# r9y9/wavenet_vocoder

Hardware: NVIDIA H100
Metric: audio samples/sec (22.05 kHz MoL, 24-layer) (higher is better)
Workload: dtype f32

## Files before the change

wavenet_vocoder_b200/csrc/wn_host.cu:

```cuda
#include <cuda_runtime.h>
#include <stdint.h>
#include <stdio.h>
#include <stdlib.h>
#include <string.h>
#include <math.h>

#include <algorithm>
#include <string>
#include <vector>

#include "../../include/wn.h"
#include "wn_plan.h"
#include "wn_kernel.cuh"
#include "wn7_plan.h"
#include "wn7_kernel.cuh"
#include "wn_aux.cuh"
#include "wn_dense.cuh"

static thread_local std::string g_err;
static int32_t fail(int32_t code, const std::string& msg) {
    g_err = msg;
    return code;
}
#define CUDA_TRY(expr)                                                                          \
// ... 108 lines not shown
    o = 0;
    pl.tb_Td = o;  o += pl.NQ_D * pl.R * 4;
    pl.tb_Sk = o;  o += pl.NQ_BS * pl.G2 * 4;
    pl.tb_sb = o;  o += 4 * pl.NQ_BS;
    pl.tb_Ha = o;  o += pl.NQ_HA * pl.S * 4;
    pl.tb_Hab = o; o += 4 * pl.NQ_HA;
    pl.tb_Hb = o;  o += pl.NQ_HB * pl.S * 4;
    pl.tb_Hbb = o; o += 4 * pl.NQ_HB;
    pl.tb_floats = align_up(o, 4);
    pl.slot_floats = align_up(std::max(pl.fb_floats, std::max(pl.L > 1 ? pl.lb_floats : 0, pl.tb_floats)), 32);
    pl.cta_w_floats = (long long)pl.fb_floats + (long long)(pl.L - 1) * pl.lb_floats + pl.tb_floats;
    pl.nblobs = pl.L + 1;
    pl.cta_cw_floats = (long long)pl.L * pl.NQ_A * pl.C * 4;

    pl.NE = pl.L + 3;
    int nc = c.exchange_copies > 0 ? c.exchange_copies : env_int("WN_NCOPY", 0);
    const int max_items = std::max(std::max(pl.NYm, pl.NXm), std::max(pl.NSm, std::max(pl.NAm, pl.NBm))) * BT;
    if (max_items > 64) return fail(WN_ERR_INVALID, "too many rows per block for this batch tile (use more blocks)");
    if (nc <= 0) nc = 1;
    nc = std::min(nc, 64 / max_items);
    pl.ncopy = std::max(1, std::min(nc, P));
    if ((pl.G2 & 1) || (pl.R & 1) || (pl.S & 1))
        return fail(WN_ERR_INVALID, "residual, gate/2 and skip channel counts must be even (16-byte exchange loads)");
    pl.ex_yx = 0;
    pl.ex_sk = pl.L * (pl.G2 + pl.R);
    pl.ex_h1 = pl.ex_sk + pl.S;
    pl.ex_h2 = pl.ex_h1 + pl.S;
    pl.ex_elems = pl.ex_h2 + pl.O;
    pl.xc_shift = env_int("WN_XC_SHIFT", 5);
    pl.xstride = env_int("WN_XSTRIDE", WN_XSTRIDE);
    pl.copy_stride_pairs = ((((long long)pl.ex_elems * BT) >> pl.xc_shift) + 2) * pl.xstride + 96;

    ringtab.assign((size_t)pl.L * std::max(pl.kw - 1, 0) * 2, 0);
    long long pos = 0;
    for (int l = 0; l < pl.L; ++l)
        for (int k = 0; k < pl.kw - 1; ++k) {
            const int D = (pl.kw - 1 - k) * wn_dilation(pl, l);
            ringtab[((size_t)l * (pl.kw - 1) + k) * 2] = (int)pos;
            ringtab[((size_t)l * (pl.kw - 1) + k) * 2 + 1] = D;
            pos += D;
        }
    pl.ring_pos_total = pos;
    const long long ring_bytes = pos * pl.RA4 * BT * 4;

    auto layout = [&](bool ring_smem) -> long long {
        long long off = 0;
        auto take = [&](long long bytes, int al) {
            off = ((off + al - 1) / al) * al;
            long long r = off;
            off += bytes;
            return (int)r;
        };
        pl.sm_bar = take((long long)(2 * pl.nblobs + 8) * 8, 16);
        pl.sm_misc = take(16, 16);
        pl.sm_in = take((long long)BT * 8 + (pl.input_kind == WN_INPUT_ONEHOT ? (long long)BT * pl.O * 4 : 0), 16);
        pl.sm_ringtab = take((long long)ringtab.size() / 2 * 3 * 4 + 16, 16);
        pl.sm_xs = take(2LL * (pl.R + pl.G2) * BT * 4, 16);
        const int nq1 = std::max(pl.NQ_A + pl.NQ_BO, std::max(pl.NQ_BS, std::max(pl.NQ_HA, pl.NQ_HB)));
        pl.red1_floats = nq1 * 4 * BT * 4 + 4;
        pl.sm_red1 = take(2LL * pl.red1_floats * 4, 16);
        pl.red2_floats = (pl.NQ_D + pl.NQ_BS + pl.NQ_BO) * 4 * BT * 4 + 4;
        pl.sm_red2 = take(2LL * pl.red2_floats * 4, 16);
        pl.sm_sb = take(2LL * pl.L * pl.RA4 * BT * 4, 16);
        pl.sm_cond = take(pl.C > 0 ? 2LL * pl.L * pl.RA4 * BT * 4 : 16, 16);
        pl.sm_skipacc = take((long long)(pl.NSm * BT + 8 * pl.NQ_BS) * 4 + 16, 16);
        pl.sm_hs = take((long long)pl.O * BT * 4, 16);
        pl.sm_noise = take((long long)BT * (pl.O + 2) * 4, 16);
        pl.sm_first = take(2LL * pl.R * 4, 16);
        pl.sm_ring = take(ring_smem ? ring_bytes : 16, 16);
        pl.sm_slots = take(0, 128);
        return off;
    };
    const long long slot_bytes = (long long)pl.slot_floats * 4;
    const int want_ring_smem = env_int("WN_RING_SMEM", -1);
    bool ring_smem = (want_ring_smem != 0) && ring_bytes <= 96 * 1024;
    long long fixed = layout(ring_smem);
    long long fit = (smem_cap - fixed) / slot_bytes;
    if (ring_smem && want_ring_smem < 0 && fit < std::min<long long>(pl.nblobs, 3)) {
        ring_smem = false;
        fixed = layout(false);
        fit = (smem_cap - fixed) / slot_bytes;
    }
    pl.ring_in_smem = ring_smem ? 1 : 0;
    if (fit >= pl.nblobs) {
        pl.nres = pl.nblobs;
        pl.nring = 0;
    } else {
        if (fit < 2) return fail(WN_ERR_INVALID, "shared memory too small for two weight slots (use more blocks)");
        int nr = c.ring_slots > 0 ? c.ring_slots : env_int("WN_RING_SLOTS", 4);
        nr = (int)std::max<long long>(2, std::min<long long>(nr, fit));
        pl.nring = nr;
        pl.nres = (int)fit - nr;
        const int force_res = env_int("WN_RESIDENT", -1);
        if (force_res >= 0 && force_res < pl.nres) pl.nres = force_res;
    }
    pl.smem_bytes = (int)(pl.sm_slots + (long long)(pl.nres + pl.nring) * slot_bytes);
    if (pl.smem_bytes > smem_cap) return fail(WN_ERR_INVALID, "shared memory map exceeds the per-block limit");
    return WN_OK;
}

static void fill_work(const wn_config& c, wn_plan_info* out) {
    const int64_t R = c.residual_channels, G = c.gate_channels, G2 = G / 2, S = c.skip_channels, O = c.out_channels;
    const int64_t L = c.layers, kw = c.kernel_size, C = c.cin_channels;
    const int64_t cin0 = (c.input_kind == WN_INPUT_SCALAR) ? 1 : O;
    const int64_t mac = cin0 * R + L * (G * kw * R + G * C + S * G2 + R * G2) + S * S + O * S;
    const int64_t biases = R + L * (G + S + R) + S + O;
    out->flops_per_sample = 2 * mac;
    out->weight_bytes_per_step = 4 * (mac + biases);
}

static void fill_info(const wn_config& c, const WnPlan& pl, wn_plan_info* out) {
    memset(out, 0, sizeof(*out));
    out->num_ctas = pl.P;
    out->threads_per_cta = WN_NTHREADS;
    out->batch_tile = pl.BT;
    out->rows_y = pl.NYm;
    out->rows_x = pl.NXm;
    out->rows_skip = pl.NSm;
    out->rows_head_a = pl.NAm;
    out->rows_head_b = pl.NBm;
// ... 1580 lines not shown
```

wavenet_vocoder_b200/csrc/wn_kernel.cuh:

```cuda
#pragma once
#include <cuda_runtime.h>
#include <stdint.h>
#include <math.h>
#include "wn_plan.h"

struct WnPtrs {
    const float* wpack;
    const float* cwpack;
    const float* gbias;
    const float* first_w;
    const float* first_b;
    uint2* xbuf;
    float* ring_g;
    const int* ringtab;
    int* err;
    const float* c;
    const float* initial;
    const float* initial_dense;
    const int* initial_rows;
    const float* test_scalar;
    const int* test_index;
    const float* test_dense;
    const float* u1;
    const float* u2;
// ... 167 lines not shown
            for (int i = 0; i < NV / 2; ++i) {
                if (i < n) {
                    const float send = hi ? v[i] : v[i + n];
                    const float keep = hi ? v[i + n] : v[i];
                    v[i] = keep + __shfl_xor_sync(0xffffffffu, send, off);
                }
            }
        } else {
            v[0] += __shfl_xor_sync(0xffffffffu, v[0], off);
        }
    }
}

__host__ __device__ constexpr int ilog2c(int v) { return v <= 1 ? 0 : 1 + ilog2c(v >> 1); }

__device__ __forceinline__ uint4 philox4(uint4 ctr, uint2 key) {
#pragma unroll
    for (int r = 0; r < 10; ++r) {
        const uint32_t hi0 = __umulhi(0xD2511F53u, ctr.x), lo0 = 0xD2511F53u * ctr.x;
        const uint32_t hi1 = __umulhi(0xCD9E8D57u, ctr.z), lo1 = 0xCD9E8D57u * ctr.z;
        ctr = make_uint4(hi1 ^ ctr.y ^ key.x, lo1, hi0 ^ ctr.w ^ key.y, lo0);
        key.x += 0x9E3779B9u;
        key.y += 0xBB67AE85u;
    }
    return ctr;
}
__device__ __forceinline__ float u01(uint32_t r) {
    const float u = ((r >> 8) + 0.5f) * (1.0f / 16777216.0f);
    return 1e-5f + u * (1.0f - 2e-5f);
}


__device__ __noinline__ long long wn_check_abort(volatile int* s_abort, int* err, long long timeout, uint32_t what,
                                                 int p, long long t0) {
    if (*s_abort) return -1;
    if (ld_flag(err) != 0) {
        *s_abort = 1;
        return -1;
    }
    const long long now = clock64();
    if (t0 == 0) return now;
    if (now - t0 > timeout) {
        if (atomicCAS(err, 0, 1) == 0) {
            err[1] = (int)what;
            err[2] = p;
            err[3] = (int)threadIdx.x;
        }
        *s_abort = 1;
        return -1;
    }
    return t0;
}

#define WN_PROF_SLOTS 96
enum { WN_PC_ACQ, WN_PC_POLL, WN_PC_STASH, WN_PC_FMA, WN_PC_READY, WN_PC_REDUCE, WN_PC_STORE, WN_PC_BAR, WN_PC_FIN,
       WN_PC_PUB, WN_PC_DDONE, WN_PC_HEAD, WN_PC_TAIL, WN_PC_CRIT };
enum { WN_PD_WAIT, WN_PD_UNSTASH, WN_PD_GEMV, WN_PD_BAR, WN_PD_FIN, WN_PD_REST, WN_PC_DEF };
enum { WN_PS_SKEW = 4 * WN_PC_CRIT, WN_PS_DEF = WN_PS_SKEW + 6, WN_PS_TMA = WN_PS_DEF + 4 * WN_PC_DEF,
       WN_PS_COND = WN_PS_TMA + 2 };
static_assert(WN_PS_COND + 2 <= WN_PROF_SLOTS, "stage profile slots");
#ifdef WN_STAGE_PROF
#define WN_PROF_DECL(N) const bool prof_ = (pp.prof != nullptr) && lane == 0; long long pc_[N] = {}, tc_ = 0;
#define WN_PROF_START() if (prof_) tc_ = clock64();
#define WN_TICK(i) if (prof_) { const long long now_ = clock64(); pc_[i] += now_ - tc_; tc_ = now_; }
#define WN_TICK_AFTER(i, sink, v) if (prof_) { *reinterpret_cast<volatile float*>(sink) = (v); } WN_TICK(i)
#define WN_PROF_STORE(base, N) if (prof_) { for (int i_ = 0; i_ < (N); ++i_) pp.prof[(size_t)p * WN_PROF_SLOTS + (base) + i_] = pc_[i_]; }
#else
#define WN_PROF_DECL(N)
#define WN_PROF_START()
#define WN_TICK(i)
#define WN_TICK_AFTER(i, sink, v)
#define WN_PROF_STORE(base, N)
#endif

#define WN_NTC 128
#define WN_GW 4
#define WN_DISPATCH_E(EV, ...)                                \
    switch (EV) {                                             \
        case 1: { constexpr int E = 1; __VA_ARGS__ } break;   \
        case 2: { constexpr int E = 2; __VA_ARGS__ } break;   \
        case 4: { constexpr int E = 4; __VA_ARGS__ } break;   \
        default: { constexpr int E = 8; __VA_ARGS__ } break;  \
    }

template <int BT, int ER, int EG, bool STREAM = false>
struct Engine {
    static constexpr int NV = 4 * BT;
    static constexpr int NA = (BT >= 8) ? 1 : 2;
    const WnPlan& pl;
    const WnPtrs& pp;
    unsigned char* sm;
    int tid, warp, lane, p;
    int gt, gw;
    uint64_t *bar_full, *bar_empty, *bar_cfull, *bar_cempty;
    volatile int* s_abort;
    volatile int* s_stash_cnt;
    volatile int* s_ddone_cnt;
    int* ringtab;
    float *xs, *ys, *red1, *red2, *sb, *pre, *cond, *skipacc, *hs, *noise, *first, *slots;
    volatile float* ring;
    float* s_in;
    int* s_idx;
    float* s_dense;
    bool dead;

    __device__ Engine(const WnPlan& pl_, const WnPtrs& pp_, unsigned char* sm_)
        : pl(pl_), pp(pp_), sm(sm_) {
        lane = threadIdx.x & 31;
        warp = pp.warp_reverse ? (WN_NTHREADS / 32 - 1) - (int)(threadIdx.x >> 5) : (int)(threadIdx.x >> 5);
        tid = warp * 32 + lane;
        p = blockIdx.x;
        gt = tid & (WN_NTC - 1);
        gw = warp & (WN_GW - 1);
        const int nslots = pl.nres + pl.nring;
        bar_full = reinterpret_cast<uint64_t*>(sm + pl.sm_bar);
        bar_empty = bar_full + nslots;
        bar_cfull = bar_empty + (pl.nring > 0 ? pl.nring : 1);
        bar_cempty = bar_cfull + 2;
        s_abort = reinterpret_cast<volatile int*>(sm + pl.sm_misc);
        s_stash_cnt = s_abort + 1;
        s_ddone_cnt = s_abort + 2;
        s_in = reinterpret_cast<float*>(sm + pl.sm_in);
        s_idx = reinterpret_cast<int*>(s_in + BT);
        s_dense = reinterpret_cast<float*>(s_idx + BT);
        ringtab = reinterpret_cast<int*>(sm + pl.sm_ringtab);
        xs = reinterpret_cast<float*>(sm + pl.sm_xs);
        ys = xs + 2 * pl.R * BT;
        red1 = reinterpret_cast<float*>(sm + pl.sm_red1);
        red2 = reinterpret_cast<float*>(sm + pl.sm_red2);
        sb = reinterpret_cast<float*>(sm + pl.sm_sb);
        pre = sb + (size_t)pl.L * pl.RA4 * BT;
        cond = reinterpret_cast<float*>(sm + pl.sm_cond);
        skipacc = reinterpret_cast<float*>(sm + pl.sm_skipacc);
        hs = reinterpret_cast<float*>(sm + pl.sm_hs);
        noise = reinterpret_cast<float*>(sm + pl.sm_noise);
        first = reinterpret_cast<float*>(sm + pl.sm_first);
        slots = reinterpret_cast<float*>(sm + pl.sm_slots);
        if (pl.ring_in_smem)
            ring = reinterpret_cast<volatile float*>(sm + pl.sm_ring);
        else
            ring = pp.ring_g + (size_t)p * pl.ring_pos_total * pl.RA4 * BT;
        dead = false;
    }

    __device__ __forceinline__ bool check_abort(uint32_t what, long long& t0) {
        t0 = wn_check_abort(s_abort, pp.err, pp.timeout_cycles, what, p, t0);
        return t0 < 0;
    }
    template <bool relaxed = false>
    __device__ __forceinline__ bool wait_bar(uint64_t* bar, uint32_t parity, uint32_t what) {
        uint32_t spins = 0;
        long long t0 = 0;
        while (!mbar_try_wait(bar, parity)) {
            if (relaxed) __nanosleep(64);
            if (((++spins) & (relaxed ? 63u : 255u)) == 0 && check_abort(what, t0)) return false;
        }
        return true;
    }
    template <bool relaxed = false>
    __device__ __forceinline__ void wait_count(volatile int* cnt, int need, uint32_t what) {
        uint32_t spins = 0;
        long long t0 = 0;
        while (*cnt < need) {
            if (relaxed) __nanosleep(32);
            if (((++spins) & (relaxed ? 63u : 255u)) == 0 && check_abort(what, t0)) {
                dead = true;
                return;
            }
        }
        __threadfence_block();
    }

    template <int E>
    __device__ __forceinline__ int elem(int j) const {
        if constexpr (BT == 1 && (E % 2) == 0) return 2 * gt + 2 * WN_NTC * (j >> 1) + (j & 1);
        else return gt + j * WN_NTC;
    }
    template <int E>
    __device__ __forceinline__ uint32_t load_vec(const uint2* __restrict__ src, int e0, int K, uint32_t tag,
                                                 float (&x)[E][BT]) {
        uint32_t bad = 0;
        if constexpr (BT == 1 && (E % 2) == 0) {
            uint4 raw[E / 2];
#pragma unroll
            for (int j = 0; j < E / 2; ++j) {
                const int k = elem<E>(2 * j);
                raw[j] = make_uint4(0u, tag, 0u, tag);
                if (k < K) raw[j] = ld_pair2(src + wn_pair_index((long long)(e0 + k)));
            }
#pragma unroll
            for (int j = 0; j < E / 2; ++j) {
                bad |= (raw[j].y ^ tag) | ((elem<E>(2 * j) + 1 < K) ? (raw[j].w ^ tag) : 0u);
                x[2 * j][0] = __uint_as_float(raw[j].x);
                x[2 * j + 1][0] = __uint_as_float(raw[j].z);
            }
        } else {
#pragma unroll
            for (int j = 0; j < E; ++j) {
                const int k = elem<E>(j);
                if (k < K) {
                    const uint2* s = src + wn_pair_index((long long)(e0 + k) * BT);
                    if constexpr (BT == 1) {
                        const uint2 v = ld_pair(s);
                        x[j][0] = __uint_as_float(v.x);
                        bad |= v.y ^ tag;
                    } else {
#pragma unroll
                        for (int b = 0; b < BT; b += 2) {
                            const uint4 v = ld_pair2(s + b);
                            x[j][b] = __uint_as_float(v.x);
                            bad |= v.y ^ tag;
                            x[j][b + 1] = __uint_as_float(v.z);
                            bad |= v.w ^ tag;
                        }
                    }
                } else {
#pragma unroll
                    for (int b = 0; b < BT; ++b) x[j][b] = 0.f;
                }
            }
        }
        return bad;
    }
    static constexpr bool WARP_POLL = BT == 1;
    __device__ __forceinline__ static bool poll_all(bool mine) {
        if constexpr (WARP_POLL) return __all_sync(0xffffffffu, mine);
        else return mine;
    }
    __device__ __forceinline__ static bool poll_any(bool mine) {
        if constexpr (WARP_POLL) return __any_sync(0xffffffffu, mine);
        else return mine;
    }
    template <int E>
    __device__ __forceinline__ void poll_vec(const uint2* __restrict__ src, int e0, int K, uint32_t tag,
                                             float (&x)[E][BT]) {
        uint32_t spins = 0;
        long long t0 = 0;
        while (!poll_all(load_vec<E>(src, e0, K, tag, x) == 0)) {
            if (((++spins) & 63u) == 0 && poll_any(check_abort(tag, t0))) {
                dead = true;
                return;
            }
        }
    }
    template <int EA, int EB>
    __device__ __forceinline__ void poll_vec2(const uint2* __restrict__ src, int ea, int KA, float (&a)[EA][BT],
                                              int eb, int KB, float (&b)[EB][BT], uint32_t tag) {
        uint32_t spins = 0;
        long long t0 = 0;
        while (true) {
            const uint32_t bad = load_vec<EA>(src, ea, KA, tag, a) | load_vec<EB>(src, eb, KB, tag, b);
            if (poll_all(bad == 0)) return;
            if (((++spins) & 63u) == 0 && poll_any(check_abort(tag, t0))) {
                dead = true;
                return;
            }
        }
    }
    template <int E>
    __device__ __forceinline__ void stash(float* dst, int K, const float (&x)[E][BT]) {
#pragma unroll
        for (int j = 0; j < E; ++j) {
            const int k = elem<E>(j);
            if (k < K) {
#pragma unroll
                for (int b = 0; b < BT; ++b) dst[k * BT + b] = x[j][b];
            }
        }
    }
    template <int E>
    __device__ __forceinline__ void unstash(const float* src, int K, float (&x)[E][BT]) {
#pragma unroll
        for (int j = 0; j < E; ++j) {
            const int k = elem<E>(j);
#pragma unroll
            for (int b = 0; b < BT; ++b) x[j][b] = (k < K) ? src[k * BT + b] : 0.f;
        }
// ... 193 lines not shown
                    const int ch = lane + 32 * i;
                    ct[b][i] = (b < B && ch < C) ? __ldg(pp.c + ((size_t)b * T + t) * C + ch) : 0.f;
                }
            float* dst = cond + (size_t)par * L * pl.RA4 * BT;
            for (int l = 0; l < L; ++l) {
                for (int q = 0; q < pl.NQ_A; ++q) {
                    float acc[NV];
#pragma unroll
                    for (int v = 0; v < NV; ++v) acc[v] = 0.f;
                    const float* wq = cw + ((size_t)(l * pl.NQ_A + q) * C) * 4;
#pragma unroll
                    for (int i = 0; i < WN_MAX_CI; ++i) {
                        const int ch = lane + 32 * i;
                        if (ch < C) {
                            const float4 w4 = __ldg(reinterpret_cast<const float4*>(wq + (size_t)ch * 4));
#pragma unroll
                            for (int b = 0; b < BT; ++b) {
                                acc[0 * BT + b] = fmaf(w4.x, ct[b][i], acc[0 * BT + b]);
                                acc[1 * BT + b] = fmaf(w4.y, ct[b][i], acc[1 * BT + b]);
                                acc[2 * BT + b] = fmaf(w4.z, ct[b][i], acc[2 * BT + b]);
                                acc[3 * BT + b] = fmaf(w4.w, ct[b][i], acc[3 * BT + b]);
                            }
                        }
                    }
                    reduce_scatter<NV>(acc, lane);
                    if ((lane & ((32 >> M) - 1)) == 0) {
                        const int v = lane >> (5 - M);
                        dst[((size_t)l * pl.RA4 + q * 4 + v / BT) * BT + (v % BT)] = acc[0];
                    }
                }
            }
            __syncwarp();
            if (lane == 0) mbar_arrive(&bar_cfull[par]);
        }
#ifdef WN_STAGE_PROF
        if (pp.prof != nullptr && lane == 0) {
            pp.prof[(size_t)p * WN_PROF_SLOTS + WN_PS_COND] = t_wait;
            pp.prof[(size_t)p * WN_PROF_SLOTS + WN_PS_COND + 1] = clock64() - t_begin;
        }
#endif
    }

    __device__ __forceinline__ void warp_argmax(float& best, int& bi) {
#pragma unroll
        for (int off = 16; off >= 1; off >>= 1) {
            const float ob = __shfl_xor_sync(0xffffffffu, best, off);
            const int oi = __shfl_xor_sync(0xffffffffu, bi, off);
            if (ob > best || (ob == best && oi < bi)) {
                best = ob;
                bi = oi;
            }
        }
    }
    __device__ void fetch_noise(int t, int b) {
        float* nz = noise + (size_t)b * (pl.O + 2);
        const int B = pp.Btot, K = pl.Kmix, O = pl.O;
        const uint32_t ub = (uint32_t)(pp.b0 + b);
        const bool replay = pp.noise_kind == 0;
        const uint2 key = make_uint2((uint32_t)pp.seed, (uint32_t)(pp.seed >> 32));
        const uint32_t tc = (STREAM ? pp.t_base : 0u) + (uint32_t)t;
        if (b >= pp.B) {
            for (int i = lane; i < O + 2; i += 32) nz[i] = 0.5f;
            return;
        }
        if (pl.head_kind == 2) {
            for (int i = lane; i < O; i += 32) {
                float e;
                if (replay) e = pp.e ? __ldg(pp.e + ((size_t)t * B + b) * O + i) : 1.0f;
                else {
                    const uint4 r = philox4(make_uint4(tc, ub, (uint32_t)i, 2u), key);
                    e = -logf(u01(r.x));
                }
                nz[i] = e;
            }
            return;
        }
        const bool mix = (pl.head_kind == 0) || (K > 1);
        if (mix) {
            for (int i = lane; i < K; i += 32) {
                float u;
                if (replay) u = __ldg(pp.u1 + ((size_t)t * B + b) * K + i);
                else u = u01(philox4(make_uint4(tc, ub, (uint32_t)i, 0u), key).x);
                nz[i] = u;
            }
        }
        if (lane == 0) {
            float v;
            if (pl.head_kind == 0) {
                if (replay) v = __ldg(pp.u2 + (size_t)t * B + b);
                else v = u01(philox4(make_uint4(tc, ub, 0u, 1u), key).x);
            } else {
                if (replay) v = __ldg(pp.z + (size_t)t * B + b);
                else {
                    const uint4 r = philox4(make_uint4(tc, ub, 0u, 1u), key);
                    v = sqrtf(-2.f * logf(u01(r.x))) * cospif(2.f * u01(r.y));
                }
            }
            nz[K] = v;
        }
    }
    __device__ void sample_utt(int t, int b) {
        const int O = pl.O, K = pl.Kmix, T = pp.T;
        const float* nz = noise + (size_t)b * (pl.O + 2);
        const bool writer = (p == 0);
        if (pl.head_kind == 2) {
            const bool softmax = (pp.flags & WN_FLAG_SOFTMAX_) != 0, quant = (pp.flags & WN_FLAG_QUANTIZE_) != 0;
            if (softmax) {
                float m = -INFINITY;
                for (int i = lane; i < O; i += 32) m = fmaxf(m, hs[i * BT + b]);
#pragma unroll
                for (int off = 16; off >= 1; off >>= 1) m = fmaxf(m, __shfl_xor_sync(0xffffffffu, m, off));
                float s = 0.f;
                for (int i = lane; i < O; i += 32) {
                    const float e = expf(hs[i * BT + b] - m);
                    hs[i * BT + b] = e;
                    s += e;
                }
#pragma unroll
                for (int off = 16; off >= 1; off >>= 1) s += __shfl_xor_sync(0xffffffffu, s, off);
                for (int i = lane; i < O; i += 32) hs[i * BT + b] = hs[i * BT + b] / s;
            }
            if (quant) {
                float sp = 0.f;
                for (int i = lane; i < O; i += 32) sp += hs[i * BT + b];
#pragma unroll
                for (int off = 16; off >= 1; off >>= 1) sp += __shfl_xor_sync(0xffffffffu, sp, off);
                float best = -INFINITY;
                int bi = 0x7fffffff;
                for (int i = lane; i < O; i += 32) {
                    const float r = (hs[i * BT + b] / sp) / nz[i];
                    if (r > best) {
                        best = r;
                        bi = i;
                    }
                }
                warp_argmax(best, bi);
                if (bi >= O) bi = 0;
                if (lane == 0) {
                    if (writer && b < pp.B) pp.out_index[(size_t)b * T + t] = bi;
                    s_idx[b] = (t + 1 < pp.T_test && b < pp.B) ? (pp.test_index ? pp.test_index[(size_t)b * pp.T_test + t + 1] : -1)
                                                               : bi;
                }
            } else {
                for (int i = lane; i < O; i += 32) {
                    const float v = hs[i * BT + b];
                    if (writer && b < pp.B) pp.out_dense[((size_t)b * O + i) * T + t] = v;
                    s_dense[b * O + i] = v;
                }
                if (lane == 0)
                    s_idx[b] = (t + 1 < pp.T_test && b < pp.B && pp.test_index)
                                   ? pp.test_index[(size_t)b * pp.T_test + t + 1] : -1;
            }
            if (t + 1 < pp.T_test && pp.test_dense != nullptr && b < pp.B) {
                for (int i = lane; i < O; i += 32)
                    s_dense[b * O + i] = pp.test_dense[((size_t)b * pp.T_test + t + 1) * O + i];
                if (lane == 0) s_idx[b] = -1;
// ... 87 lines not shown
            if (pl.C > 0) v += cd[idx];
            for (int k = 0; k < kw - 1; ++k) {
                const int e = (l * (kw - 1) + k) * 3;
                int pos = ringtab[e + 2];
                if (t > 0) { ++pos; if (pos == ringtab[e + 1]) pos = 0; }
                v += ring[((size_t)ringtab[e] + pos) * RA4 * BT + rr * BT + b];
            }
            pre[idx] = v;
        }
        __syncwarp();
        if (pl.C > 0) {
            if (lane == 0) mbar_arrive(&bar_cempty[t & 1]);
        }
    }

    __device__ void crit_loop() {
        const int L = pl.L, R = pl.R, G2 = pl.G2, S = pl.S, O = pl.O, T = pp.T, P = pl.P, ncopy = pl.ncopy;
        int y0, ny, x0r, nx, s0, ns, a0, na, b0, nb;
        wn_part(G2, P, p, y0, ny);
        wn_part(R, P, p, x0r, nx);
        wn_part(S, P, p, s0, ns);
        wn_part(S, P, p, a0, na);
        wn_part(O, P, p, b0, nb);
        const int ES = efor(S), EO = efor(O);
        const uint2* xin = pp.xbuf + (size_t)(p % ncopy) * pl.copy_stride_pairs;
        const uint32_t NEID = (uint32_t)L + 3u;
        const int YX = G2 + R;
        const float RSQRT2 = 0.70710678118654752440f;
        const int NQ_A = pl.NQ_A, NQ_BO = pl.NQ_BO, nqc = NQ_A + NQ_BO;
        const int fl = gt & 63;
        const bool grpA = gt < 64;
        auto role = [&](int nitems, int& item, int& copy) {
            item = -1; copy = 0;
            if (nitems > 0 && fl < nitems * ncopy) { item = fl % nitems; copy = fl / nitems; }
        };
        int it_y, cp_y, it_x, cp_x, it_s, cp_s, it_a, cp_a, it_b, cp_b;
        role(ny * BT, it_y, cp_y);
        role(nx * BT, it_x, cp_x);
        role(ns * BT, it_s, cp_s);
        role(na * BT, it_a, cp_a);
        role(nb * BT, it_b, cp_b);
        if (!grpA) it_y = it_s = it_a = it_b = -1;
        if (grpA) it_x = -1;
        const int pa_idx = it_y >= 0 ? (2 * (it_y / BT)) * BT + (it_y % BT) : 0;
        float xr[ER][BT], yr[EG][BT];
        WN_PROF_DECL(WN_PC_CRIT)
#ifdef WN_STAGE_PROF
        volatile uint32_t* s_arrive = reinterpret_cast<volatile uint32_t*>(bar_full + 2 * pl.nblobs + 4);
        long long skew = 0, nskew = 0, nlast[WN_GW] = {};
#endif
        int nstash = 0;
        int ndone = 0;
        long long t_pub = clock64();
        if (bar_groups(false)) return;

        for (int t = 0; t < T; ++t) {
            const uint32_t tagbase = (uint32_t)t * NEID + 1u;
            WN_PROF_START();
            bool step_dead = false;
            do {
                make_x0(xr);
                WN_TICK(WN_PC_TAIL);
                {
                    const float* W = acquire_blob(t, 0);
                    float pre_a = 0.f, pre_b = 0.f;
                    if (it_y >= 0) { pre_a = pre[pa_idx]; pre_b = pre[pa_idx + BT]; }
                    float* r1 = red1;
                    gemv<ER>(W + pl.fb_Zx, NQ_A, R, xr, r1);
                    if (bar_or_n<1, WN_NTC>(dead)) { step_dead = true; break; }
                    if (it_y >= 0) {
                        const int fr = it_y / BT, fb = it_y % BT;
                        const float a = red_sum(r1, 2 * fr, fb) + pre_a;
                        const float g = red_sum(r1, 2 * fr + 1, fb) + pre_b;
                        publish(pl.ex_yx + y0 + fr, fb, cp_y, gate(a, g), tagbase + wn_eid_yx(0));
                    }
                    release_blob(t, 0);
                    t_pub = clock64();
                    WN_TICK(WN_PC_HEAD);
                }
                for (int s = 1; s < L; ++s) {
                    const float* W = acquire_blob(t, s);
                    float pre_a = 0.f, pre_b = 0.f;
                    if (it_y >= 0) { pre_a = pre[pa_idx + s * pl.RA4 * BT]; pre_b = pre[pa_idx + s * pl.RA4 * BT + BT]; }
                    float4 wp[NPRE_A];
                    if constexpr (NPRE > 0) preload0(W, NQ_A, nqc, wp);
                    WN_TICK(WN_PC_ACQ);
                    {
                        const int e0 = pl.ex_yx + (s - 1) * YX;
                        const uint32_t tag = tagbase + wn_eid_yx(s - 1);
                        if (pp.gate_cycles > 0) { while (clock64() - t_pub < pp.gate_cycles) {} }
                        if (s >= 2) poll_vec2<EG, ER>(xin, e0, G2, yr, e0 + G2, R, xr, tag);
                        else poll_vec<EG>(xin, e0, G2, tag, yr);
                    }
                    WN_TICK(WN_PC_POLL);
                    float* xst = xs + (size_t)(s & 1) * R * BT;
                    float* r1 = red1 + (size_t)(s & 1) * pl.red1_floats;
                    stash<ER>(xst, R, xr);
                    stash<EG>(ys + (size_t)(s & 1) * G2 * BT, G2, yr);
                    WN_TICK(WN_PC_STASH);
                    for (int q = 0; q < nqc; q += NA) {
                        float acc[NA][NV];
                        if (NPRE > 0 && q == 0) {
                            pass0(W, NQ_A, nqc, wp, yr, xr, acc);
                        } else {
#pragma unroll
                            for (int h = 0; h < NA; ++h) {
#pragma unroll
                                for (int v = 0; v < NV; ++v) acc[h][v] = 0.f;
                                const int qq = q + h;
                                if (qq < NQ_A) {
                                    quad_fma<EG>(W + pl.lb_Zy + (size_t)qq * G2 * 4, G2, yr, acc[h]);
                                    quad_fma<ER>(W + pl.lb_Zx + (size_t)qq * R * 4, R, xr, acc[h]);
                                } else if (qq < nqc) {
                                    quad_fma<EG>(W + pl.lb_Xo + (size_t)(qq - NQ_A) * G2 * 4, G2, yr, acc[h]);
                                }
                            }
                        }
                        WN_TICK(WN_PC_FMA);
                        WN_TICK_AFTER(WN_PC_READY, r1 + (size_t)q * NV * WN_GW + gw, acc[NA - 1][NV - 1]);
                        reduce_scatter_multi<NA, NV>(acc, lane);
                        WN_TICK(WN_PC_REDUCE);
#pragma unroll
                        for (int h = 0; h < NA; ++h)
                            if (q + h < nqc) quad_store(acc[h], q + h, r1);
                        WN_TICK(WN_PC_STORE);
                    }
#ifdef WN_STAGE_PROF
                    if (prof_) s_arrive[(s & 1) * WN_GW + gw] = (uint32_t)tc_;
#endif
                    if (bar_or_n<1, WN_NTC>(dead)) { step_dead = true; break; }
                    WN_TICK(WN_PC_BAR);
// ... 34 lines not shown
                    if (it_x >= 0) publish(pl.ex_yx + s * YX + G2 + x0r + it_x / BT, it_x % BT, cp_x, vx, tag);
                    release_blob(t, s);
                    t_pub = clock64();
                    WN_TICK(WN_PC_PUB);
                    if (s >= 2) { wait_count(s_ddone_cnt, WN_GW * (ndone + 1), 0x08000000u); ++ndone; }
                    WN_TICK(WN_PC_DDONE);
                }
                if (step_dead) break;
                const float* H = acquire_blob(t, L);
                {
                    const int e0 = pl.ex_yx + (L - 1) * YX;
                    const uint32_t tag = tagbase + wn_eid_yx(L - 1);
                    if (L >= 2) poll_vec2<EG, ER>(xin, e0, G2, yr, e0 + G2, R, xr, tag);
                    else poll_vec<EG>(xin, e0, G2, tag, yr);
                }
                stash<ER>(xs + (size_t)(L & 1) * R * BT, R, xr);
                float* r1 = red1 + (size_t)(L & 1) * pl.red1_floats;
                gemv<EG>(H + pl.tb_Sk, pl.NQ_BS, G2, yr, r1);
                if (bar_or_n<1, WN_NTC>(dead)) { step_dead = true; break; }
                if (gt == WN_NTC - 1) {
                    __threadfence_block();
                    *s_stash_cnt = nstash + 1;
                }
                ++nstash;
                if (L >= 2) { wait_count(s_ddone_cnt, WN_GW * (ndone + 1), 0x08000001u); ++ndone; }
                if (it_s >= 0) {
                    const int fr = it_s / BT, fb = it_s % BT;
                    float tot = red_sum(r1, fr, fb) + H[pl.tb_sb + fr];
                    if (L >= 2) tot = skipacc[it_s] + tot;
                    publish(pl.ex_sk + s0 + fr, fb, cp_s, fmaxf(tot * pl.skip_scale, 0.f), tagbase + wn_eid_sk(pl));
                }
                float* r1a = red1 + (size_t)((L + 1) & 1) * pl.red1_floats;
                if (na > 0) {
                    WN_DISPATCH_E(ES, { float h[E][BT];
                                        poll_vec<E>(xin, pl.ex_sk, S, tagbase + wn_eid_sk(pl), h);
                                        gemv<E>(H + pl.tb_Ha, pl.NQ_HA, S, h, r1a); });
                }
                if (bar_or_n<1, WN_NTC>(dead)) { step_dead = true; break; }
                if (it_a >= 0) {
                    const int fr = it_a / BT, fb = it_a % BT;
                    publish(pl.ex_h1 + a0 + fr, fb, cp_a, fmaxf(red_sum(r1a, fr, fb) + H[pl.tb_Hab + fr], 0.f), tagbase + wn_eid_h1(pl));
                }
                if (nb > 0) {
                    WN_DISPATCH_E(ES, { float h[E][BT];
                                        poll_vec<E>(xin, pl.ex_h1, S, tagbase + wn_eid_h1(pl), h);
                                        gemv<E>(H + pl.tb_Hb, pl.NQ_HB, S, h, r1); });
                }
                if (bar_or_n<1, WN_NTC>(dead)) { step_dead = true; break; }
                if (it_b >= 0) {
                    const int fr = it_b / BT, fb = it_b % BT;
                    publish(pl.ex_h2 + b0 + fr, fb, cp_b, red_sum(r1, fr, fb) + H[pl.tb_Hbb + fr], tagbase + wn_eid_h2(pl));
                }
                release_blob(t, L);
                {
                    WN_DISPATCH_E(EO, { float h[E][BT];
                                        poll_vec<E>(xin, pl.ex_h2, O, tagbase + wn_eid_h2(pl), h);
                                        stash<E>(hs, O, h); });
                }
                WN_TICK(WN_PC_HEAD);
            } while (false);
            if (bar_groups(dead || step_dead)) return;
            if (L >= 1) ++ndone;
            step_tail(t);
            if (bar_groups(false)) return;
            WN_TICK(WN_PC_TAIL);
        }
        WN_PROF_STORE(gw * WN_PC_CRIT, WN_PC_CRIT)
#ifdef WN_STAGE_PROF
        if (prof_ && gw == 0) {
            long long* out = pp.prof + (size_t)p * WN_PROF_SLOTS;
            out[WN_PS_SKEW] = skew;
            out[WN_PS_SKEW + 1] = nskew;
            for (int w = 0; w < WN_GW; ++w) out[WN_PS_SKEW + 2 + w] = nlast[w];
        }
#endif
    }

    __device__ __forceinline__ void step_tail(int t) {
        const int O = pl.O, T = pp.T;
        if (p == 0 && pp.params_out != nullptr) {
            for (int i = tid; i < O * BT; i += WN_NT) {
                const int o = i / BT, b = i % BT;
                if (b < pp.B) pp.params_out[((size_t)b * O + o) * T + t] = hs[i];
            }
            if (pl.head_kind == 2) bar_groups(false);
        }
        if (warp < BT) {
            sample_utt(t, warp);
#ifndef WN_NO_SAMPLER_SYNCWARP
            __syncwarp();
#endif
            if (t + 1 < T) fetch_noise(t + 1, warp);
        }
        for (int i = WN_NT - 1 - tid; i < pl.L * (pl.kw - 1); i += WN_NT) {
            const int pos = ringtab[i * 3 + 2] + 1;
            ringtab[i * 3 + 2] = (pos == ringtab[i * 3 + 1]) ? 0 : pos;
        }
    }

    __device__ void def_loop() {
        const int L = pl.L, R = pl.R, G2 = pl.G2, T = pp.T, P = pl.P, kw = pl.kw;
        int s0, ns;
        wn_part(pl.S, P, p, s0, ns);
        const int NQ_D = pl.NQ_D, NQ_BS = pl.NQ_BS, nqd = (kw > 1 ? NQ_D : 0) + NQ_BS;
        const int qoff = (kw > 1 ? NQ_D : 0);
        const int nring_items = (kw - 1) * pl.RA * BT, nskip_items = ns * BT;
        float xr[ER][BT], yr[EG][BT];
        WN_PROF_DECL(WN_PC_DEF)
        int nstash = 0;

        auto stage = [&](int t, int s, int layer, const float* Td, const float* Sk, const float* skb) {
            wait_count<true>(s_stash_cnt, nstash + 1, 0x04000000u);
            ++nstash;
            WN_TICK(WN_PD_WAIT);
            unstash<ER>(xs + (size_t)(s & 1) * R * BT, R, xr);
            if (Sk) unstash<EG>(ys + (size_t)(s & 1) * G2 * BT, G2, yr);
            WN_TICK(WN_PD_UNSTASH);
            float* red = red2 + (size_t)(s & 1) * pl.red2_floats;
            const int nq = Sk ? nqd : qoff;
            for (int q = 0; q < nq; q += NA) {
                float acc[NA][NV];
#pragma unroll
                for (int h = 0; h < NA; ++h) {
#pragma unroll
                    for (int v = 0; v < NV; ++v) acc[h][v] = 0.f;
                    const int qq = q + h;
                    if (qq < qoff) quad_fma<ER>(Td + (size_t)qq * R * 4, R, xr, acc[h]);
                    else if (qq < nq) quad_fma<EG>(Sk + (size_t)(qq - qoff) * G2 * 4, G2, yr, acc[h]);
                }
                reduce_scatter_multi<NA, NV>(acc, lane);
#pragma unroll
                for (int h = 0; h < NA; ++h)
                    if (q + h < nq) quad_store(acc[h], q + h, red);
            }
            WN_TICK(WN_PD_GEMV);
            const bool d = bar_or_n<2, WN_NTC>(dead);
            WN_TICK(WN_PD_BAR);
            if (!d) {
                for (int f = gt; f < nring_items; f += WN_NTC) {
                    const int dr = f / BT, db = f % BT, tap = dr / pl.RA, rr = dr % pl.RA;
                    const int e = (layer * (kw - 1) + tap) * 3;
                    ring[((size_t)ringtab[e] + ringtab[e + 2]) * pl.RA4 * BT + rr * BT + db] = red_sum(red, dr, db);
                }
                if (Sk) {
                    for (int f = gt; f < nskip_items; f += WN_NTC) {
                        const int fr = f / BT, fb = f % BT;
                        const float h = red_sum(red, qoff * 4 + fr, fb) + skb[fr];
                        skipacc[f] = (layer == 0) ? h : skipacc[f] + h;
                    }
                }
            }
            __threadfence_block();
            __syncwarp();
            if (lane == 0) atomicAdd((int*)s_ddone_cnt, 1);
            WN_TICK(WN_PD_FIN);
            return d;
        };

        build_pre(0);
        if (bar_groups(dead)) return;
        for (int t = 0; t < T; ++t) {
            WN_PROF_START();
            bool step_dead = false;
            release_blob(t, 0);
            for (int s = 1; s < L && !step_dead; ++s) {
                const float* W = acquire_blob(t, s);
                step_dead = stage(t, s, s - 1, W + pl.lb_Td, W + pl.lb_Sk, W + pl.lb_sb);
                release_blob(t, s);
            }
            if (!step_dead) {
                const float* H = acquire_blob(t, L);
                step_dead = stage(t, L, L - 1, H + pl.tb_Td, nullptr, nullptr);
                release_blob(t, L);
            }
            if (!step_dead && t + 1 < T) {
                if (bar_or_n<2, WN_NTC>(dead)) step_dead = true;
                else build_pre(t + 1);
            }
            if (bar_groups(dead || step_dead)) return;
            step_tail(t);
            if (bar_groups(false)) return;
            WN_TICK(WN_PD_REST);
        }
        WN_PROF_STORE(WN_PS_DEF + gw * WN_PC_DEF, WN_PC_DEF)
    }
};

template <int BT>
__device__ __noinline__ void wn_store_state(const WnPlan& pl, const WnPtrs& pp, unsigned char* sm) {
    const int warp = pp.warp_reverse ? (WN_NTHREADS / 32 - 1) - (int)(threadIdx.x >> 5) : (int)(threadIdx.x >> 5);
    const int tid = warp * 32 + (int)(threadIdx.x & 31), p = blockIdx.x;
    if (tid >= WN_NT) return;
    const long long ring_n = wn_state_ring_floats(pl);
    if (pl.ring_in_smem) {
        const volatile float* ring = reinterpret_cast<const volatile float*>(sm + pl.sm_ring);
        float* dst = pp.state + (size_t)p * ring_n;
        for (long long i = tid; i < ring_n; i += WN_NT) dst[i] = ring[i];
    }
    if (p == 0) {
        const float* s_in = reinterpret_cast<const float*>(sm + pl.sm_in);
        const int* s_idx = reinterpret_cast<const int*>(s_in + BT);
        const float* s_dense = reinterpret_cast<const float*>(s_idx + BT);
        float* fb = pp.state + (size_t)pl.P * ring_n;
        for (int b = tid; b < BT; b += WN_NT) {
            fb[b] = s_in[b];
            fb[BT + b] = __int_as_float(s_idx[b]);
        }
        if (pl.input_kind != 0)
            for (int i = tid; i < BT * pl.O; i += WN_NT) fb[2 * BT + i] = s_dense[i];
    }
}

template <int BT, int ER, int EG, bool STREAM = false>
__global__ void __launch_bounds__(WN_NTHREADS, 1)
wn_persistent_kernel(const __grid_constant__ WnPlan pl, const __grid_constant__ WnPtrs pp) {
    extern __shared__ __align__(1024) unsigned char smem_raw[];
    Engine<BT, ER, EG, STREAM> eng(pl, pp, smem_raw);
    const int tid = eng.tid, p = blockIdx.x;
    const int nslots = pl.nres + pl.nring;
    if (tid == 0) {
        for (int i = 0; i < nslots; ++i) mbar_init(&eng.bar_full[i], 1);
        for (int i = 0; i < pl.nring; ++i) mbar_init(&eng.bar_empty[i], WN_NWARP);
        for (int i = 0; i < 2; ++i) {
            mbar_init(&eng.bar_cfull[i], 1);
            mbar_init(&eng.bar_cempty[i], WN_GW);
        }
        *eng.s_abort = 0;
        *eng.s_stash_cnt = 0;
        *eng.s_ddone_cnt = 0;
        asm volatile("fence.mbarrier_init.release.cluster;" ::: "memory");
    }
    const long long ring_n = wn_state_ring_floats(pl);
    if (pl.ring_in_smem) {
        const float* src = (STREAM && pp.state_load) ? pp.state + (size_t)p * ring_n : nullptr;
        for (long long i = tid; i < ring_n; i += WN_NTHREADS) eng.ring[i] = src ? src[i] : 0.f;
    }
    for (int i = tid; i < pl.NSm * BT + 4; i += WN_NTHREADS) eng.skipacc[i] = 0.f;
    for (int i = tid; i < pl.L * (pl.kw - 1); i += WN_NTHREADS) {
        eng.ringtab[i * 3] = pp.ringtab[i * 2];
        eng.ringtab[i * 3 + 1] = pp.ringtab[i * 2 + 1];
        eng.ringtab[i * 3 + 2] = STREAM ? (int)(pp.t_base % (unsigned)pp.ringtab[i * 2 + 1]) : 0;
    }
    for (int k = tid; k < pl.R; k += WN_NTHREADS) {
        eng.first[k] = (pl.input_kind == 0) ? pp.first_w[k] : 0.f;
        eng.first[pl.R + k] = pp.first_b[k];
    }
    {
        int y0, ny;
        wn_part(pl.G2, pl.P, p, y0, ny);
        const float* blob0 = pp.wpack + (size_t)p * pl.cta_w_floats;
        const int n = pl.L * pl.RA4 * BT;
        for (int i = tid; i < n; i += WN_NTHREADS) {
            const int b = i % BT, rr = (i / BT) % pl.RA4, l = i / (BT * pl.RA4);
            float v = 0.f;
            if (rr < pl.RA && (rr >> 1) < ny) {
                v = blob0[wn_blob_off(pl, l) + (l == 0 ? pl.fb_zb : pl.lb_zb) + rr];
                if (pp.gbias != nullptr && b < pp.B) {
                    const int grow = (rr & 1) ? pl.G2 + y0 + (rr >> 1) : y0 + (rr >> 1);
                    v += pp.gbias[((size_t)b * pl.L + l) * pl.G + grow];
                }
            }
            eng.sb[i] = v;
        }
    }
    if (tid < BT) {
        const int b = tid;
        float v = 0.f;
        int idx = -1;
        if (b < pp.B) {
            if (pl.input_kind == 0) {
                if (pp.T_test > 0) v = pp.test_scalar[(size_t)b * pp.T_test];
                else if (pp.initial) v = pp.initial[b];
            } else {
                if (pp.T_test > 0) idx = pp.test_index ? pp.test_index[(size_t)b * pp.T_test] : -1;
                else if (pp.initial_dense) idx = -1;
                else if (pp.initial_rows) idx = pp.initial_rows[b];
                else idx = pp.initial_index;
            }
        } else if (pl.input_kind != 0) idx = 0;
        const float* fb = (STREAM && pp.state_load) ? pp.state + (size_t)pl.P * ring_n : nullptr;
        eng.s_in[b] = fb ? fb[b] : v;
        eng.s_idx[b] = fb ? __float_as_int(fb[BT + b]) : idx;
    }
    if (pl.input_kind != 0) {
        const float* dsrc = nullptr;
        size_t stride = 0;
        if (pp.T_test > 0 && pp.test_dense != nullptr) { dsrc = pp.test_dense; stride = (size_t)pp.T_test * pl.O; }
        else if (pp.T_test == 0 && pp.initial_dense != nullptr) { dsrc = pp.initial_dense; stride = (size_t)pl.O; }
        const float* fb = (STREAM && pp.state_load) ? pp.state + (size_t)pl.P * ring_n + 2 * BT : nullptr;
        for (int i = tid; i < BT * pl.O; i += WN_NTHREADS) {
            const int b = i / pl.O, o = i % pl.O;
            eng.s_dense[i] = fb ? fb[i] : ((dsrc && b < pp.B) ? dsrc[(size_t)b * stride + o] : 0.f);
        }
    }
    const int warp = tid >> 5;
    if (warp < BT && warp < WN_NWARP) eng.fetch_noise(0, warp);
    __syncthreads();
    if (warp == WN_NWARP) {
        eng.tma_loop();
        return;
    }
    if (warp == WN_NWARP + 1) {
        if (pl.C > 0) eng.cond_loop();
        return;
    }
    if (warp < WN_GW) eng.crit_loop();
    else eng.def_loop();
    if constexpr (STREAM) wn_store_state<BT>(pl, pp, smem_raw);
}

__global__ void wn_gbias_kernel(const float* __restrict__ wg, const float* __restrict__ g, float* __restrict__ out,
                                int L, int G, int gin) {
    const int l = blockIdx.x, b = blockIdx.y;
    for (int row = threadIdx.x; row < G; row += blockDim.x) {
        const float* w = wg + ((size_t)l * G + row) * gin;
        float a = 0.f;
        for (int i = 0; i < gin; ++i) a = fmaf(w[i], g[(size_t)b * gin + i], a);
        out[((size_t)b * L + l) * G + row] = a;
    }
}

__global__ void wn_sample_kernel(const float* __restrict__ y, int B, int O, int T, const float* __restrict__ u1,
                                 const float* __restrict__ n2, float* __restrict__ out, int gauss) {
    const int i = blockIdx.x * blockDim.x + threadIdx.x;
    if (i >= B * T) return;
    const int b = i / T, t = i % T;
    const float* yb = y + (size_t)b * O * T + t;
    float mean, ls;
    const int K = (O == 2) ? 1 : O / 3;
    if (K > 1 || (!gauss)) {
        float best = -INFINITY;
        int bi = 0;
        for (int k = 0; k < K; ++k) {
            const float gk = yb[(size_t)k * T] - logf(-logf(u1[((size_t)t * B + b) * K + k]));
            if (gk > best) {
                best = gk;
                bi = k;
            }
        }
        mean = yb[(size_t)(K + bi) * T];
        ls = yb[(size_t)(2 * K + bi) * T];
    } else if (O == 2) {
        mean = yb[0];
        ls = yb[(size_t)T];
    } else {
        mean = yb[(size_t)T];
        ls = yb[(size_t)2 * T];
    }
    const float v = n2[(size_t)t * B + b];
    float xv;
    if (!gauss) xv = __fadd_rn(mean, __fmul_rn(expf(ls), __fsub_rn(logf(v), logf(__fsub_rn(1.0f, v)))));
    else xv = __fadd_rn(__fmul_rn(v, expf(ls)), mean);
    out[i] = fminf(fmaxf(xv, -1.0f), 1.0f);
}

}
```

Before: 16990.

## Decouple critical and deferred warp groups with counters and double-buffered noise

Replaces the full-block barriers around the per-step tail with group-local named barriers and shared-memory counters. The deferred group now signals pre-activation readiness and draws next-step noise into a double-buffered noise area during its layer loop. The critical group waits on those counters and samples. Ring position updates move to the deferred group only. It also enables warp-level polling for one specific configuration and adds profiling slots. The aim is to remove whole-block synchronisation from the serial per-sample critical path, at the cost of more subtle ordering between the groups and more shared memory for noise.

```diff
diff --git a/wavenet_vocoder_b200/csrc/wn_host.cu b/wavenet_vocoder_b200/csrc/wn_host.cu
--- a/wavenet_vocoder_b200/csrc/wn_host.cu
+++ b/wavenet_vocoder_b200/csrc/wn_host.cu
@@ -184,7 +184,7 @@
             return (int)r;
         };
         pl.sm_bar = take((long long)(2 * pl.nblobs + 8) * 8, 16);
-        pl.sm_misc = take(16, 16);
+        pl.sm_misc = take(32, 16);
         pl.sm_in = take((long long)BT * 8 + (pl.input_kind == WN_INPUT_ONEHOT ? (long long)BT * pl.O * 4 : 0), 16);
         pl.sm_ringtab = take((long long)ringtab.size() / 2 * 3 * 4 + 16, 16);
         pl.sm_xs = take(2LL * (pl.R + pl.G2) * BT * 4, 16);
@@ -197,7 +197,7 @@
         pl.sm_cond = take(pl.C > 0 ? 2LL * pl.L * pl.RA4 * BT * 4 : 16, 16);
         pl.sm_skipacc = take((long long)(pl.NSm * BT + 8 * pl.NQ_BS) * 4 + 16, 16);
         pl.sm_hs = take((long long)pl.O * BT * 4, 16);
-        pl.sm_noise = take((long long)BT * (pl.O + 2) * 4, 16);
+        pl.sm_noise = take(2LL * BT * (pl.O + 2) * 4, 16);
         pl.sm_first = take(2LL * pl.R * 4, 16);
         pl.sm_ring = take(ring_smem ? ring_bytes : 16, 16);
         pl.sm_slots = take(0, 128);
diff --git a/wavenet_vocoder_b200/csrc/wn_kernel.cuh b/wavenet_vocoder_b200/csrc/wn_kernel.cuh
--- a/wavenet_vocoder_b200/csrc/wn_kernel.cuh
+++ b/wavenet_vocoder_b200/csrc/wn_kernel.cuh
@@ -243,10 +243,12 @@
     return t0;
 }
 
-#define WN_PROF_SLOTS 96
+#define WN_PROF_SLOTS 160
 enum { WN_PC_ACQ, WN_PC_POLL, WN_PC_STASH, WN_PC_FMA, WN_PC_READY, WN_PC_REDUCE, WN_PC_STORE, WN_PC_BAR, WN_PC_FIN,
-       WN_PC_PUB, WN_PC_DDONE, WN_PC_HEAD, WN_PC_TAIL, WN_PC_CRIT };
-enum { WN_PD_WAIT, WN_PD_UNSTASH, WN_PD_GEMV, WN_PD_BAR, WN_PD_FIN, WN_PD_REST, WN_PC_DEF };
+       WN_PC_PUB, WN_PC_DDONE, WN_PC_HEAD, WN_PC_H2, WN_PC_SBAR1, WN_PC_SAMPLE, WN_PC_NOISE, WN_PC_RING, WN_PC_SBAR2,
+       WN_PC_PREW, WN_PC_X0, WN_PC_CRIT };
+enum { WN_PD_WAIT, WN_PD_UNSTASH, WN_PD_GEMV, WN_PD_BAR, WN_PD_FIN, WN_PD_PRE, WN_PD_SBAR1, WN_PD_SAMPLE, WN_PD_NOISE,
+       WN_PD_RING, WN_PD_SBAR2, WN_PC_DEF };
 enum { WN_PS_SKEW = 4 * WN_PC_CRIT, WN_PS_DEF = WN_PS_SKEW + 6, WN_PS_TMA = WN_PS_DEF + 4 * WN_PC_DEF,
        WN_PS_COND = WN_PS_TMA + 2 };
 static_assert(WN_PS_COND + 2 <= WN_PROF_SLOTS, "stage profile slots");
@@ -287,6 +289,8 @@
     volatile int* s_abort;
     volatile int* s_stash_cnt;
     volatile int* s_ddone_cnt;
+    volatile int* s_pre_cnt;
+    volatile int* s_noise_cnt;
     int* ringtab;
     float *xs, *ys, *red1, *red2, *sb, *pre, *cond, *skipacc, *hs, *noise, *first, *slots;
     volatile float* ring;
@@ -311,6 +315,8 @@
         s_abort = reinterpret_cast<volatile int*>(sm + pl.sm_misc);
         s_stash_cnt = s_abort + 1;
         s_ddone_cnt = s_abort + 2;
+        s_pre_cnt = s_abort + 3;
+        s_noise_cnt = s_abort + 4;
         s_in = reinterpret_cast<float*>(sm + pl.sm_in);
         s_idx = reinterpret_cast<int*>(s_in + BT);
         s_dense = reinterpret_cast<float*>(s_idx + BT);
@@ -413,7 +419,7 @@
         }
         return bad;
     }
-    static constexpr bool WARP_POLL = BT == 1;
+    static constexpr bool WARP_POLL = BT == 1 || (BT == 4 && ER == 4 && EG == 2 && !STREAM);
     __device__ __forceinline__ static bool poll_all(bool mine) {
         if constexpr (WARP_POLL) return __all_sync(0xffffffffu, mine);
         else return mine;
@@ -713,8 +719,11 @@
             }
         }
     }
+    __device__ __forceinline__ float* noise_row(int t, int b) const {
+        return noise + ((size_t)(t & 1) * BT + b) * (pl.O + 2);
+    }
     __device__ void fetch_noise(int t, int b) {
-        float* nz = noise + (size_t)b * (pl.O + 2);
+        float* nz = noise_row(t, b);
         const int B = pp.Btot, K = pl.Kmix, O = pl.O;
         const uint32_t ub = (uint32_t)(pp.b0 + b);
         const bool replay = pp.noise_kind == 0;
@@ -762,7 +771,7 @@
     }
     __device__ void sample_utt(int t, int b) {
         const int O = pl.O, K = pl.Kmix, T = pp.T;
-        const float* nz = noise + (size_t)b * (pl.O + 2);
+        const float* nz = noise_row(t, b);
         const bool writer = (p == 0);
         if (pl.head_kind == 2) {
             const bool softmax = (pp.flags & WN_FLAG_SOFTMAX_) != 0, quant = (pp.flags & WN_FLAG_QUANTIZE_) != 0;
@@ -956,15 +965,17 @@
         int nstash = 0;
         int ndone = 0;
         long long t_pub = clock64();
-        if (bar_groups(false)) return;
+        const bool hs_warp0 = BT == 1 && O <= 32;
+        const int ndraw = BT < WN_GW ? BT : WN_GW;
 
         for (int t = 0; t < T; ++t) {
             const uint32_t tagbase = (uint32_t)t * NEID + 1u;
             WN_PROF_START();
             bool step_dead = false;
             do {
+                wait_count(s_pre_cnt, t + 1, 0x08000002u);
+                WN_TICK(WN_PC_PREW);
                 make_x0(xr);
-                WN_TICK(WN_PC_TAIL);
                 {
                     const float* W = acquire_blob(t, 0);
                     float pre_a = 0.f, pre_b = 0.f;
@@ -980,7 +991,7 @@
                     }
                     release_blob(t, 0);
                     t_pub = clock64();
-                    WN_TICK(WN_PC_HEAD);
+                    WN_TICK(WN_PC_X0);
                 }
                 for (int s = 1; s < L; ++s) {
                     const float* W = acquire_blob(t, s);
@@ -1121,18 +1132,29 @@
                     publish(pl.ex_h2 + b0 + fr, fb, cp_b, red_sum(r1, fr, fb) + H[pl.tb_Hbb + fr], tagbase + wn_eid_h2(pl));
                 }
                 release_blob(t, L);
+                WN_TICK(WN_PC_HEAD);
                 {
                     WN_DISPATCH_E(EO, { float h[E][BT];
                                         poll_vec<E>(xin, pl.ex_h2, O, tagbase + wn_eid_h2(pl), h);
                                         stash<E>(hs, O, h); });
                 }
-                WN_TICK(WN_PC_HEAD);
+                WN_TICK(WN_PC_H2);
             } while (false);
-            if (bar_groups(dead || step_dead)) return;
+            if (hs_warp0) {
+                if (step_dead) return;
+                __syncwarp();
+            } else if (bar_or_n<1, WN_NTC>(dead || step_dead)) {
+                return;
+            }
+            WN_TICK(WN_PC_SBAR1);
             if (L >= 1) ++ndone;
-            step_tail(t);
-            if (bar_groups(false)) return;
-            WN_TICK(WN_PC_TAIL);
+            if (gw < BT) {
+                wait_count(s_noise_cnt, ndraw * t, 0x08000003u);
+                for (int b = gw; b < BT; b += WN_GW) sample_step(t, b);
+            }
+            WN_TICK(WN_PC_SAMPLE);
+            if (bar_or_n<1, WN_NTC>(dead)) return;
+            WN_TICK(WN_PC_SBAR2);
         }
         WN_PROF_STORE(gw * WN_PC_CRIT, WN_PC_CRIT)
 #ifdef WN_STAGE_PROF
@@ -1145,26 +1167,12 @@
 #endif
     }
 
-    __device__ __forceinline__ void step_tail(int t) {
-        const int O = pl.O, T = pp.T;
-        if (p == 0 && pp.params_out != nullptr) {
-            for (int i = tid; i < O * BT; i += WN_NT) {
-                const int o = i / BT, b = i % BT;
-                if (b < pp.B) pp.params_out[((size_t)b * O + o) * T + t] = hs[i];
-            }
-            if (pl.head_kind == 2) bar_groups(false);
-        }
-        if (warp < BT) {
-            sample_utt(t, warp);
-#ifndef WN_NO_SAMPLER_SYNCWARP
+    __device__ __forceinline__ void sample_step(int t, int b) {
+        if (p == 0 && pp.params_out != nullptr && b < pp.B) {
+            for (int o = lane; o < pl.O; o += 32) pp.params_out[((size_t)b * pl.O + o) * pp.T + t] = hs[o * BT + b];
             __syncwarp();
-#endif
-            if (t + 1 < T) fetch_noise(t + 1, warp);
-        }
-        for (int i = WN_NT - 1 - tid; i < pl.L * (pl.kw - 1); i += WN_NT) {
-            const int pos = ringtab[i * 3 + 2] + 1;
-            ringtab[i * 3 + 2] = (pos == ringtab[i * 3 + 1]) ? 0 : pos;
-        }
+        }
+        sample_utt(t, b);
     }
 
     __device__ void def_loop() {
@@ -1226,8 +1234,26 @@
             return d;
         };
 
+        const int ndraw = BT < WN_GW ? BT : WN_GW;
+        auto draw_noise = [&](int t) {
+            if (gw < ndraw && t < T) {
+                for (int b = gw; b < BT; b += WN_GW) fetch_noise(t, b);
+                __threadfence_block();
+                __syncwarp();
+                if (lane == 0) atomicAdd((int*)s_noise_cnt, 1);
+            }
+            WN_TICK(WN_PD_NOISE);
+        };
+        auto pre_ready = [&](int t) {
+            if (gt == WN_NTC - 1) {
+                __threadfence_block();
+                *s_pre_cnt = t + 1;
+            }
+        };
+
         build_pre(0);
-        if (bar_groups(dead)) return;
+        if (bar_or_n<2, WN_NTC>(dead)) return;
+        pre_ready(0);
         for (int t = 0; t < T; ++t) {
             WN_PROF_START();
             bool step_dead = false;
@@ -1236,20 +1262,27 @@
                 const float* W = acquire_blob(t, s);
                 step_dead = stage(t, s, s - 1, W + pl.lb_Td, W + pl.lb_Sk, W + pl.lb_sb);
                 release_blob(t, s);
+                if (s == 1) draw_noise(t + 1);
             }
             if (!step_dead) {
                 const float* H = acquire_blob(t, L);
                 step_dead = stage(t, L, L - 1, H + pl.tb_Td, nullptr, nullptr);
                 release_blob(t, L);
+                if (L == 1) draw_noise(t + 1);
             }
             if (!step_dead && t + 1 < T) {
                 if (bar_or_n<2, WN_NTC>(dead)) step_dead = true;
                 else build_pre(t + 1);
             }
-            if (bar_groups(dead || step_dead)) return;
-            step_tail(t);
-            if (bar_groups(false)) return;
-            WN_TICK(WN_PD_REST);
+            WN_TICK(WN_PD_PRE);
+            if (bar_or_n<2, WN_NTC>(dead || step_dead)) return;
+            WN_TICK(WN_PD_SBAR1);
+            pre_ready(t + 1);
+            for (int i = gt; i < L * (kw - 1); i += WN_NTC) {
+                const int pos = ringtab[i * 3 + 2] + 1;
+                ringtab[i * 3 + 2] = (pos == ringtab[i * 3 + 1]) ? 0 : pos;
+            }
+            WN_TICK(WN_PD_RING);
         }
         WN_PROF_STORE(WN_PS_DEF + gw * WN_PC_DEF, WN_PC_DEF)
     }
@@ -1297,6 +1330,8 @@
         *eng.s_abort = 0;
         *eng.s_stash_cnt = 0;
         *eng.s_ddone_cnt = 0;
+        *eng.s_pre_cnt = 0;
+        *eng.s_noise_cnt = 0;
         asm volatile("fence.mbarrier_init.release.cluster;" ::: "memory");
     }
     const long long ring_n = wn_state_ring_floats(pl);
@@ -1375,7 +1410,10 @@
     }
     if (warp < WN_GW) eng.crit_loop();
     else eng.def_loop();
-    if constexpr (STREAM) wn_store_state<BT>(pl, pp, smem_raw);
+    if constexpr (STREAM) {
+        bar_groups(false);
+        wn_store_state<BT>(pl, pp, smem_raw);
+    }
 }
 
 __global__ void wn_gbias_kernel(const float* __restrict__ wg, const float* __restrict__ g, float* __restrict__ out,
```

After: 17300, median of 6. +1.8%, better.
